# CESSProject/DeOSS

Measured on AMD Instinct MI355X. Metric: device-resident GiB/s hashed to Merkle root; 1/2/4/8 MI355X scaling, higher is better.
Workload: dtype u32; 1 GPU; BASELINE configs[1]: 1 object of 8 GiB (8589934592 B) in 1 chunk-range shard(s) of 8 GiB, chunk 33554432 B (256 leaves); object_bytes=8589934592, chunk=33554432, leaves=256, parallelism=single GPU

## Files before the change

deoss_amd/csrc/merkle_kernels.hpp:

```cpp
#pragma once
#include "quad_ring.hpp"
#include "sha256_gfx950.hpp"

namespace dm {

constexpr int kBlock = 256;
constexpr int kLeafFuseMax = 8;
constexpr int kReduceTile = 512;

struct LeafArgs {
    const uint8_t* base;
    uint64_t pitch;
    uint64_t leaf_len;
    uint64_t last_len;
    const uint64_t* addrs;
    const uint64_t* lens;
    uint64_t nleaves;
    uint64_t byte_off;
    uint64_t byte_end;
    uint32_t* state;
    uint8_t* digests;
    uint8_t* level_out;
    uint32_t fuse_levels;
};
// ... 368 lines not shown
        X7 = t_ + dpp_swap_pairs(y_);                                                  \
    } while (0)

__device__ __forceinline__ void pair_rounds_from_kw(uint32_t (&x)[4], const uint4 (*kw)[kLatLeaves], uint32_t lane,
                                                    uint32_t sh1, uint32_t sh2, uint32_t sh3, uint32_t msk,
                                                    bool lane_b) {
    uint32_t x4 = x[0], x5 = x[1], x6 = x[2], x7 = x[3];
    uint4 q = kw[0][lane];
#pragma unroll
    for (int g = 0; g < 16; g++) {
        uint4 nq = q;
        if (g + 1 < 16) nq = kw[g + 1][lane];
        DM_PAIR_ROUND(x4, x5, x6, x7, q.x);
        DM_PAIR_ROUND(x7, x4, x5, x6, q.y);
        DM_PAIR_ROUND(x6, x7, x4, x5, q.z);
        DM_PAIR_ROUND(x5, x6, x7, x4, q.w);
        q = nq;
    }
    x[0] += x4; x[1] += x5; x[2] += x6; x[3] += x7;
}

template <bool TABLE, bool ALIGNED>
__global__ __launch_bounds__(kLatThreads) void leaf_kernel_pair(LeafArgs a) {
    __shared__ uint4 ring[kLatRing][16][kLatLeaves];
    __shared__ uint32_t lds_a[kPairLeaves][8];
    __shared__ uint32_t lds_b[kPairLeaves / 2][8];
    const uint32_t lane = threadIdx.x & (kLatLeaves - 1);
    const bool producer = __builtin_amdgcn_readfirstlane(threadIdx.x) < kLatLeaves;
    const bool lane_b = (lane & 1) != 0;
    const uint32_t c = lane >> 1;
    const uint64_t first = (uint64_t)blockIdx.x * kPairLeaves;
    const uint64_t i = first + c;
    const LeafView v = leaf_view<TABLE>(a, i);
    const uint64_t NB = wave_max_u64(v.nb);
    if (producer) {
        Blk cur;
        if (v.nb > 0 && !lane_b) cur = load_block<ALIGNED>(v.p);
        for (uint64_t b = 0; b < NB; b++) {
            if (b < v.nb) {
                uint32_t w[16];
                block_words(cur, w);
                if (b + 1 < v.nb && !lane_b) cur = load_block<ALIGNED>(v.p + 64 * (b + 1));
                uint4 (*kw)[kLatLeaves] = ring[b % kLatRing];
#pragma unroll
                for (int q = 0; q < 16; q++) {
                    uint32_t u[4];
#pragma unroll
                    for (int j = 0; j < 4; j++) {
                        const int t = 4 * q + j;
                        uint32_t wt;
                        if (t < 16) {
                            wt = w[t];
                        } else {
                            wt = ssig1(w[(t - 2) & 15]) + w[(t - 7) & 15] + ssig0(w[(t - 15) & 15]) + w[t & 15];
                            w[t & 15] = wt;
                        }
                        u[j] = lane_b ? 0u : kSha256K[t] + wt;
                    }
                    kw[q][lane] = make_uint4(u[0], u[1], u[2], u[3]);
                }
            }
            __syncthreads();
        }
        __syncthreads();
    } else {
        const uint32_t sh1 = lane_b ? 2 : 6, sh2 = lane_b ? 13 : 11, sh3 = lane_b ? 22 : 25;
        const uint32_t msk = lane_b ? 0u : ~0u;
        uint32_t st0[8];
        if (v.active) load_or_init_state(a, i, st0);
        else init_state(st0);
        uint32_t x[4];
#pragma unroll
        for (int k = 0; k < 4; k++) x[k] = lane_b ? st0[k] : st0[4 + k];
        __syncthreads();
        for (uint64_t b = 0; b < NB; b++) {
            if (b < v.nb) pair_rounds_from_kw(x, ring[b % kLatRing], lane, sh1, sh2, sh3, msk, lane_b);
            __syncthreads();
        }
        uint32_t st[8];
#pragma unroll
        for (int k = 0; k < 4; k++) {
            const uint32_t other = dpp_swap_pairs(x[k]);
            st[k] = lane_b ? x[k] : other;
            st[4 + k] = lane_b ? other : x[k];
        }
        if (v.active && !lane_b) {
            leaf_epilogue<ALIGNED>(a, i, v, st);
#pragma unroll
            for (int k = 0; k < 8; k++) lds_a[c][k] = st[k];
        }
    }
    if (a.fuse_levels == 0) return;
    __syncthreads();
    const uint32_t cnt = (uint32_t)((a.nleaves - first) < kPairLeaves ? (a.nleaves - first) : kPairLeaves);
    uint32_t (*res)[8];
    const uint32_t out_cnt = lds_reduce(lds_a, lds_b, cnt, a.fuse_levels, &res);
    if (threadIdx.x < out_cnt) {
        uint32_t o8[8];
#pragma unroll
        for (int k = 0; k < 8; k++) o8[k] = res[threadIdx.x][k];
        const uint64_t o = (uint64_t)blockIdx.x * (kPairLeaves >> a.fuse_levels) + threadIdx.x;
        store_digest(a.level_out + 32 * o, o8);
    }
}

constexpr int kQuadLeaves = 8;
constexpr int kQuadBlocks = 8;
constexpr int kQuadFuseMax = 3;
constexpr int kQuadRow = kQuadLeaves;
constexpr size_t kQuadLdsBytes = sizeof(uint4) * kLatRing * 16 * kQuadBlocks * kQuadRow + 4 * 8 * kQuadLeaves +
                                 4 * 8 * (kQuadLeaves / 2);
static_assert(4 * kQuadLdsBytes <= (160u << 10), "four compact K1Q workgroups must fit a CU's LDS");

#define DM_QS_HEAD(X4, X5, X6)                                                                   \
    "v_alignbit_b32 %[r], %[" X4 "], %[" X4 "], %[sh]\n\t"                                      \
    "v_bitop3_b32 %[f], %[" X4 "], %[" X5 "], %[msk] bitop3:0x1e\n\t"                          \
    "v_bitop3_b32 %[f], %[f], %[" X6 "], %[" X5 "] bitop3:0xca\n\t"                             \
    "v_xor_b32_dpp %[s], %[r], %[r] quad_perm:[1,2,0,3] row_mask:0xf bank_mask:0xf\n\t"
#define DM_QS_SIGMA "v_xor_b32_dpp %[s], %[r], %[s] quad_perm:[2,0,1,3] row_mask:0xf bank_mask:0xf\n\t"
#define DM_QS_STEP_Q(X4, X5, X6, X7, H, HN, VN, QP)                                             \
    DM_QS_HEAD(X4, X5, X6)                                                                       \
    "v_sub_u32_dpp %[" X6 "], %[" VN "], %[" X6 "] quad_perm:" QP " row_mask:0xf bank_mask:0x3\n\t" \
    DM_QS_SIGMA                                                                                  \
    "v_sub_u32_dpp %[" HN "], %[" X4 "], %[" X6 "] row_ror:8 row_mask:0xf bank_mask:0xf\n\t"    \
    "v_add3_u32 %[" X7 "], %[s], %[f], %[" H "]\n\t"
#define DM_QS_STEP(X4, X5, X6, X7, H, HN, VN) DM_QS_STEP_Q(X4, X5, X6, X7, H, HN, VN, "[0,1,2,3]")
#define DM_QS_STEP_A(X4, X5, X6, X7, H, HN)                                                     \
    DM_QS_HEAD(X4, X5, X6)                                                                       \
    DM_QS_SIGMA                                                                                  \
    "v_sub_u32_dpp %[" HN "], %[" X4 "], %[" X6 "] row_ror:8 row_mask:0xf bank_mask:0xf\n\t"    \
    "v_add3_u32 %[" X7 "], %[s], %[f], %[" H "]\n\t"
#define DM_QS_STEP_END(X4, X5, X6, X7, H)                                                       \
    DM_QS_HEAD(X4, X5, X6)                                                                       \
    DM_QS_SIGMA                                                                                  \
    "v_add3_u32 %[" X7 "], %[s], %[f], %[" H "]\n\t"
#define DM_QS_STEPS4V(V0, V1, V2, V3)                                                          \
    DM_QS_STEP("a", "b", "c", "d", "h", "g", V0) DM_QS_STEP("d", "a", "b", "c", "g", "h", V1)   \
    DM_QS_STEP("c", "d", "a", "b", "h", "g", V2) DM_QS_STEP("b", "c", "d", "a", "g", "h", V3)
#define DM_QS_ALIGN_MIS ".p2align 3\n\t.if %[mis]\n\ts_nop 0\n\t.endif\n\t"
#define DM_QS_PROLOGUE(V) DM_QS_PROLOGUE_AT(V, DM_QS_ALIGN_MIS, "[0,1,2,3]")
#define DM_QS_PROLOGUE_AT(V, ALIGN, QP)                                                           \
    "s_nop 1\n\t" ALIGN                                                                          \
    "v_sub_u32_dpp %[d], %[" V "], %[d] quad_perm:" QP " row_mask:0xf bank_mask:0x3\n\t"         \
    "v_sub_u32_dpp %[h], %[b], %[d] row_ror:8 row_mask:0xf bank_mask:0xf\n\t"
#define DM_QS_RESTORE_A(P, X) "v_mov_b32_dpp %[" P "], %[" X "] quad_perm:[0,1,2,3] row_mask:0xf bank_mask:0xc\n\t"
#define DM_QS_GROUP0(V0, V1, V2, V3)                                                             \
    DM_QS_STEP("a", "b", "c", "d", "h", "g", V0) DM_QS_RESTORE_A("d", "x3")                      \
    DM_QS_STEP("d", "a", "b", "c", "g", "h", V1) DM_QS_RESTORE_A("c", "x2")                      \
    DM_QS_STEP("c", "d", "a", "b", "h", "g", V2) DM_QS_STEP("b", "c", "d", "a", "g", "h", V3)
#define DM_QS_FF(X, P, BANKS) "v_add_u32_dpp %[" X "], %[" P "], %[" X "] quad_perm:[0,1,2,3] row_mask:0xf bank_mask:" BANKS "\n\t"
#define DM_QS_TAIL(V0, V1, V2)                                                                   \
    DM_QS_STEP("a", "b", "c", "d", "h", "g", V0) DM_QS_STEP("d", "a", "b", "c", "g", "h", V1)   \
    DM_QS_STEP("c", "d", "a", "b", "h", "g", V2) DM_QS_STEP_A("b", "c", "d", "a", "g", "h")      \
    DM_QS_FF("x3", "d", "0x3") DM_QS_FF("x2", "c", "0x3") DM_QS_FF("x1", "b", "0x3")             \
    DM_QS_FF("x0", "a", "0x3")                                                                   \
    DM_QS_STEP_A("a", "b", "c", "d", "h", "g") DM_QS_STEP_END("d", "a", "b", "c", "g")           \
    DM_QS_FF("x0", "a", "0xc") DM_QS_FF("x1", "b", "0xc") DM_QS_FF("x3", "d", "0xc")             \
    DM_QS_FF("x2", "c", "0xc")
#define DM_QS_STEPS4Q(V0, Q0, V1, Q1, V2, Q2, V3, Q3)                                          \
    DM_QS_STEP_Q("a", "b", "c", "d", "h", "g", V0, Q0) DM_QS_STEP_Q("d", "a", "b", "c", "g", "h", V1, Q1) \
    DM_QS_STEP_Q("c", "d", "a", "b", "h", "g", V2, Q2) DM_QS_STEP_Q("b", "c", "d", "a", "g", "h", V3, Q3)
#define DM_QS_GROUP0Q(V0, Q0, V1, Q1, V2, Q2, V3, Q3)                                          \
    DM_QS_STEP_Q("a", "b", "c", "d", "h", "g", V0, Q0) DM_QS_RESTORE_A("d", "x3")              \
    DM_QS_STEP_Q("d", "a", "b", "c", "g", "h", V1, Q1) DM_QS_RESTORE_A("c", "x2")              \
    DM_QS_STEP_Q("c", "d", "a", "b", "h", "g", V2, Q2) DM_QS_STEP_Q("b", "c", "d", "a", "g", "h", V3, Q3)
#define DM_QS_TAILQ(V0, Q0, V1, Q1, V2, Q2)                                                     \
    DM_QS_STEP_Q("a", "b", "c", "d", "h", "g", V0, Q0) DM_QS_STEP_Q("d", "a", "b", "c", "g", "h", V1, Q1) \
    DM_QS_STEP_Q("c", "d", "a", "b", "h", "g", V2, Q2) DM_QS_STEP_A("b", "c", "d", "a", "g", "h") \
    DM_QS_FF("x3", "d", "0x3") DM_QS_FF("x2", "c", "0x3") DM_QS_FF("x1", "b", "0x3")             \
    DM_QS_FF("x0", "a", "0x3")                                                                   \
    DM_QS_STEP_A("a", "b", "c", "d", "h", "g") DM_QS_STEP_END("d", "a", "b", "c", "g")           \
    DM_QS_FF("x0", "a", "0xc") DM_QS_FF("x1", "b", "0xc") DM_QS_FF("x3", "d", "0xc")             \
    DM_QS_FF("x2", "c", "0xc")
#define DM_QS_OUT                                                                                \
    : [a] "+v"(p0), [b] "+v"(p1), [c] "+v"(p2), [d] "+v"(p3), [h] "+v"(h), [g] "+v"(g),           \
      [x0] "+v"(x[0]), [x1] "+v"(x[1]), [x2] "+v"(x[2]), [x3] "+v"(x[3]), [r] "=&v"(r_),          \
      [f] "=&v"(f_), [s] "=&v"(s_)
#define DM_QS_OPS DM_QS_OUT : [mis] "i"(MIS ? 1 : 0), [sh] "v"(sh.x), [msk] "v"(msk), [v0] "v"(v0), [v1] "v"(v1), [v2] "v"(v2), [v3] "v"(v3)

template <bool MIS, class KW>
__device__ __forceinline__ void quad_block_skewed(uint32_t (&x)[4], KW kw, uint3 sh, uint32_t msk) {
    uint32_t p0 = x[0], p1 = x[1], p2 = x[2], p3 = x[3], h = 0, g = 0, r_, f_, s_;
    uint4 q = kw(0), nq = kw(1);
    {
        const uint32_t v0 = q.x, v1 = 0, v2 = 0, v3 = 0;
        asm volatile(DM_QS_PROLOGUE("v0") DM_QS_OPS);
    }
#pragma unroll
    for (int grp = 0; grp < 16; grp++) {
        const uint4 nnq = grp + 2 < 16 ? kw(grp + 2) : nq;
        const uint32_t v0 = q.y, v1 = q.z, v2 = q.w, v3 = nq.x;
        if (grp == 0) {
            asm volatile(DM_QS_ALIGN_MIS DM_QS_GROUP0("v0", "v1", "v2", "v3") DM_QS_OPS);
        } else if (grp < 15) {
            asm volatile(DM_QS_ALIGN_MIS DM_QS_STEPS4V("v0", "v1", "v2", "v3") DM_QS_OPS);
        } else {
            asm volatile(DM_QS_ALIGN_MIS DM_QS_TAIL("v0", "v1", "v2") DM_QS_OPS);
        }
        q = nq;
        nq = nnq;
    }
}

constexpr int kLgkmWait0 = 0xC07F;

#define DM_QS_HNB(HN, A, B, BANKS) "v_sub_u32_dpp %[" HN "], %[" A "], %[" B "] row_ror:8 row_mask:0xf bank_mask:" BANKS "\n\t"
#define DM_QS_ADDB(D, A, B, BANKS) "v_add_u32_dpp %[" D "], %[" A "], %[" B "] quad_perm:[0,1,2,3] row_mask:0xf bank_mask:" BANKS "\n\t"
#define DM_QS_MOVB(D, S, BANKS) "v_mov_b32_dpp %[" D "], %[" S "] quad_perm:[0,1,2,3] row_mask:0xf bank_mask:" BANKS "\n\t"
#define DM_QS_KWN(X6, S, N) "v_sub_u32_dpp %[" X6 "], %[" N "], %[" S "] quad_perm:[0,0,0,0] row_mask:0xf bank_mask:0x3\n\t"
#define DM_QS_ADD3(X7, H) "v_add3_u32 %[" X7 "], %[s], %[f], %[" H "]\n\t"
#define DM_QS_LINKQ(V0, Q0, V1, Q1, V2, Q2, N0, N1, N2)                                          \
    DM_QS_STEP_Q("a", "b", "c", "d", "h", "g", V0, Q0) DM_QS_STEP_Q("d", "a", "b", "c", "g", "h", V1, Q1) \
    DM_QS_STEP_Q("c", "d", "a", "b", "h", "g", V2, Q2)                                           \
    DM_QS_ADDB("x1", "x1", "b", "0xc") DM_QS_ADDB("x3", "x3", "d", "0x3")                        \
                                            \
    DM_QS_HEAD("b", "c", "d") DM_QS_KWN("d", "x3", N0) DM_QS_SIGMA                               \
    DM_QS_HNB("h", "x1", "d", "0x3") DM_QS_HNB("h", "b", "d", "0xc") DM_QS_ADD3("a", "g")        \
    DM_QS_ADDB("b", "x1", "b", "0x3") DM_QS_ADDB("c", "x2", "c", "0x3")                          \
    DM_QS_HNB("g", "a", "c", "0xc") DM_QS_ADDB("x0", "x0", "a", "0xc")                           \
    DM_QS_ADDB("a", "a", "x0", "0x3") DM_QS_MOVB("x2", "c", "0x3")                               \
                                                            \
    DM_QS_HEAD("a", "b", "c") DM_QS_KWN("c", "c", N1) DM_QS_SIGMA                                \
    DM_QS_HNB("g", "x0", "c", "0x3") DM_QS_ADD3("d", "h")                                        \
    DM_QS_ADDB("x3", "x3", "d", "0xc") DM_QS_MOVB("x1", "b", "0x3") DM_QS_MOVB("x0", "a", "0x3") \
                                           \
    DM_QS_HEAD("d", "a", "b") DM_QS_KWN("b", "b", N2) DM_QS_SIGMA                                \
    DM_QS_HNB("h", "x3", "b", "0x3") DM_QS_HNB("h", "d", "x1", "0xc") DM_QS_ADD3("c", "g")       \
    DM_QS_ADDB("x2", "x2", "c", "0xc") DM_QS_MOVB("a", "x0", "0xc") DM_QS_MOVB("d", "x3", "0xc") \
    DM_QS_MOVB("c", "x2", "0xc")
#define DM_QS_BODYQ                                                                              \
    DM_QS_STEPS4Q("q01", "[1,1,1,1]", "q02", "[1,1,1,1]", "q03", "[1,1,1,1]", "q00", "[2,2,2,2]") \
    DM_QS_STEPS4Q("q01", "[2,2,2,2]", "q02", "[2,2,2,2]", "q03", "[2,2,2,2]", "q00", "[3,3,3,3]") \
    DM_QS_STEPS4Q("q01", "[3,3,3,3]", "q02", "[3,3,3,3]", "q03", "[3,3,3,3]", "q10", "[0,0,0,0]") \
    DM_QS_STEPS4Q("q11", "[0,0,0,0]", "q12", "[0,0,0,0]", "q13", "[0,0,0,0]", "q10", "[1,1,1,1]") \
    DM_QS_STEPS4Q("q11", "[1,1,1,1]", "q12", "[1,1,1,1]", "q13", "[1,1,1,1]", "q10", "[2,2,2,2]") \
    DM_QS_STEPS4Q("q11", "[2,2,2,2]", "q12", "[2,2,2,2]", "q13", "[2,2,2,2]", "q10", "[3,3,3,3]") \
    DM_QS_STEPS4Q("q11", "[3,3,3,3]", "q12", "[3,3,3,3]", "q13", "[3,3,3,3]", "q20", "[0,0,0,0]") \
    DM_QS_STEPS4Q("q21", "[0,0,0,0]", "q22", "[0,0,0,0]", "q23", "[0,0,0,0]", "q20", "[1,1,1,1]") \
    DM_QS_STEPS4Q("q21", "[1,1,1,1]", "q22", "[1,1,1,1]", "q23", "[1,1,1,1]", "q20", "[2,2,2,2]") \
    DM_QS_STEPS4Q("q21", "[2,2,2,2]", "q22", "[2,2,2,2]", "q23", "[2,2,2,2]", "q20", "[3,3,3,3]") \
    DM_QS_STEPS4Q("q21", "[3,3,3,3]", "q22", "[3,3,3,3]", "q23", "[3,3,3,3]", "q30", "[0,0,0,0]") \
    DM_QS_STEPS4Q("q31", "[0,0,0,0]", "q32", "[0,0,0,0]", "q33", "[0,0,0,0]", "q30", "[1,1,1,1]") \
    DM_QS_STEPS4Q("q31", "[1,1,1,1]", "q32", "[1,1,1,1]", "q33", "[1,1,1,1]", "q30", "[2,2,2,2]") \
    DM_QS_STEPS4Q("q31", "[2,2,2,2]", "q32", "[2,2,2,2]", "q33", "[2,2,2,2]", "q30", "[3,3,3,3]")
#define DM_QS_FILLQ                                                                              \
    DM_QS_PROLOGUE_AT("q00", DM_QS_ALIGN_MIS, "[0,0,0,0]")                                       \
    DM_QS_GROUP0Q("q01", "[0,0,0,0]", "q02", "[0,0,0,0]", "q03", "[0,0,0,0]", "q00", "[1,1,1,1]")
#define DM_QS_CONTQ                                                                              \
    DM_QS_ALIGN_MIS                                                                              \
    DM_QS_STEP_Q("c", "d", "a", "b", "h", "g", "q03", "[0,0,0,0]") DM_QS_STEP_Q("b", "c", "d", "a", "g", "h", "q00", "[1,1,1,1]")
#define DM_QS_ENDLINKQ DM_QS_LINKQ("q31", "[3,3,3,3]", "q32", "[3,3,3,3]", "q33", "[3,3,3,3]", "n0", "n1", "n2")
#define DM_QS_ENDTAILQ DM_QS_TAILQ("q31", "[3,3,3,3]", "q32", "[3,3,3,3]", "q33", "[3,3,3,3]")
#define DM_QS_STATE [a] "+v"(P[0]), [b] "+v"(P[1]), [c] "+v"(P[2]), [d] "+v"(P[3]),              \
                    [x0] "+v"(x[0]), [x1] "+v"(x[1]), [x2] "+v"(x[2]), [x3] "+v"(x[3]),           \
                    [r] "=&v"(r_), [f] "=&v"(f_), [s] "=&v"(s_)
#define DM_QS_KIN [mis] "i"(MIS ? 1 : 0), [sh] "v"(sh.x), [msk] "v"(msk),                        \
                  [q00] "v"(K[0].x), [q01] "v"(K[0].y), [q02] "v"(K[0].z), [q03] "v"(K[0].w),     \
                  [q10] "v"(K[1].x), [q11] "v"(K[1].y), [q12] "v"(K[1].z), [q13] "v"(K[1].w),     \
                  [q20] "v"(K[2].x), [q21] "v"(K[2].y), [q22] "v"(K[2].z), [q23] "v"(K[2].w),     \
                  [q30] "v"(K[3].x), [q31] "v"(K[3].y), [q32] "v"(K[3].z), [q33] "v"(K[3].w)

template <bool MIS, int K8>
__device__ __forceinline__ void quad_block_regs(uint32_t (&x)[4], uint32_t (&P)[4], uint32_t& h, uint32_t& g,
                                                const uint4 (&K)[4], const uint4& N, uint3 sh, uint32_t msk) {
    uint32_t r_, f_, s_;
    if constexpr (K8 == 0) {
        asm volatile(DM_QS_FILLQ DM_QS_BODYQ DM_QS_ENDLINKQ
                     : DM_QS_STATE, [h] "=&v"(h), [g] "=&v"(g)
                     : DM_QS_KIN, [n0] "v"(N.x), [n1] "v"(N.y), [n2] "v"(N.z));
    } else if constexpr (K8 < kQuadBlocks - 1) {
        asm volatile(DM_QS_CONTQ DM_QS_BODYQ DM_QS_ENDLINKQ
                     : DM_QS_STATE, [h] "+v"(h), [g] "+v"(g)
                     : DM_QS_KIN, [n0] "v"(N.x), [n1] "v"(N.y), [n2] "v"(N.z));
    } else {
        asm volatile(DM_QS_CONTQ DM_QS_BODYQ DM_QS_ENDTAILQ
                     : DM_QS_STATE, [h] "+v"(h), [g] "+v"(g)
                     : DM_QS_KIN);
    }
}

template <int G, int ROW, bool MIS, int K8 = 0>
__device__ __forceinline__ void quad_stage_blocks(uint32_t (&x)[4], uint32_t (&P)[4], uint32_t& h, uint32_t& g,
                                                  uint4 (&S)[3][4], const uint4* kw, uint3 sh, uint32_t msk) {
    __builtin_amdgcn_s_waitcnt(kLgkmWait0);
    if constexpr (K8 + 2 < kQuadBlocks) {
#pragma unroll
        for (int t = 0; t < 4; t++) S[(K8 + 2) % 3][t] = kw[(K8 + 2) * ROW + 4 * t * G];
    }
    quad_block_regs<MIS, K8>(x, P, h, g, S[K8 % 3], S[(K8 + 1) % 3][0], sh, msk);
    if constexpr (K8 + 1 < kQuadBlocks) quad_stage_blocks<G, ROW, MIS, K8 + 1>(x, P, h, g, S, kw, sh, msk);
}
template <int G, int ROW, bool MIS>
__device__ __forceinline__ void quad_stage_regs(uint32_t (&x)[4], const uint4* kw, uint3 sh, uint32_t msk) {
    uint4 S[3][4];
    uint32_t P[4] = {x[0], x[1], x[2], x[3]}, h, g;
#pragma unroll
    for (int k = 0; k < 2; k++) {
#pragma unroll
        for (int t = 0; t < 4; t++) S[k][t] = kw[k * ROW + 4 * t * G];
    }
    quad_stage_blocks<G, ROW, MIS>(x, P, h, g, S, kw, sh, msk);
}

constexpr int kQuadWideRing = quad_ring::kWideDepth;
constexpr int kQuadSets = quad_ring::kSets;
template <int G, int ROW, int K8, bool FILL, bool TAIL, bool LOAD>
__device__ __forceinline__ void quad_xstage_block(uint32_t (&x)[4], uint32_t (&P)[4], uint32_t& h, uint32_t& g,
                                                  uint4 (&S)[kQuadSets][4], const uint4* src, uint3 sh, uint32_t msk) {
    static_assert((LOAD || !quad_ring::block_prefetches(K8, true)) && (!TAIL || !quad_ring::block_links(K8, true)) &&
                      !(FILL && TAIL) && quad_ring::prefetch_of(K8).block == (K8 + quad_ring::kAhead) % kQuadBlocks,
                  "only the last stage of a run skips a load or drains: quad_ring.hpp");
    __builtin_amdgcn_s_waitcnt(kLgkmWait0);
    if constexpr (LOAD) {
        constexpr quad_ring::BlockRef pf = quad_ring::prefetch_of(K8);
#pragma unroll
        for (int t = 0; t < 4; t++) S[quad_ring::set_of(K8 + quad_ring::kAhead)][t] = src[pf.block * ROW + 4 * t * G];
    }
    quad_block_regs<false, FILL ? 0 : TAIL ? kQuadBlocks - 1 : 1>(x, P, h, g, S[quad_ring::set_of(K8)],
                                                                 S[quad_ring::set_of(K8 + 1)][0], sh, msk);
}
template <int G, int ROW>
__device__ __forceinline__ uint32_t quad_run_xstage(uint32_t (&x)[4], const uint4* colp, uint32_t slot, uint64_t n,
                                                    uint3 sh, uint32_t msk) {
    uint4 S[kQuadSets][4];
    uint32_t P[4] = {x[0], x[1], x[2], x[3]}, h, g;
    const uint4* cur = colp + slot * 16 * G;
#pragma unroll
    for (int k = 0; k < quad_ring::kAhead; k++) {
#pragma unroll
        for (int t = 0; t < 4; t++) S[k][t] = cur[k * ROW + 4 * t * G];
    }
    quad_xstage_block<G, ROW, 0, true, false, true>(x, P, h, g, S, cur, sh, msk);
    for (uint64_t s = 1; s < n; s++) {
        slot = quad_ring::next_slot(slot, kQuadWideRing);
        const uint4* nxt = colp + slot * 16 * G;
        quad_xstage_block<G, ROW, 1, false, false, true>(x, P, h, g, S, cur, sh, msk);
        quad_xstage_block<G, ROW, 2, false, false, true>(x, P, h, g, S, cur, sh, msk);
        quad_xstage_block<G, ROW, 3, false, false, true>(x, P, h, g, S, cur, sh, msk);
        quad_xstage_block<G, ROW, 4, false, false, true>(x, P, h, g, S, cur, sh, msk);
        quad_xstage_block<G, ROW, 5, false, false, true>(x, P, h, g, S, cur, sh, msk);
        quad_xstage_block<G, ROW, 6, false, false, true>(x, P, h, g, S, nxt, sh, msk);
        quad_xstage_block<G, ROW, 7, false, false, true>(x, P, h, g, S, nxt, sh, msk);
        __syncthreads();
        quad_xstage_block<G, ROW, 0, false, false, true>(x, P, h, g, S, nxt, sh, msk);
        cur = nxt;
    }
    quad_xstage_block<G, ROW, 1, false, false, true>(x, P, h, g, S, cur, sh, msk);
    quad_xstage_block<G, ROW, 2, false, false, true>(x, P, h, g, S, cur, sh, msk);
    quad_xstage_block<G, ROW, 3, false, false, true>(x, P, h, g, S, cur, sh, msk);
    quad_xstage_block<G, ROW, 4, false, false, true>(x, P, h, g, S, cur, sh, msk);
    quad_xstage_block<G, ROW, 5, false, false, true>(x, P, h, g, S, cur, sh, msk);
    quad_xstage_block<G, ROW, 6, false, false, false>(x, P, h, g, S, cur, sh, msk);
    quad_xstage_block<G, ROW, 7, false, true, false>(x, P, h, g, S, cur, sh, msk);
    __syncthreads();
    return quad_ring::next_slot(slot, kQuadWideRing);
}

template <bool ALIGNED, int G>
__device__ __forceinline__ void quad_produce_block(const LeafView& v, Blk& cur, uint64_t b, uint4* kw) {
    if (b >= v.nb) return;
    uint32_t w[16];
    block_words(cur, w);
    if (b + kQuadBlocks < v.nb) cur = load_block<ALIGNED>(v.p + 64 * (b + kQuadBlocks));
#pragma unroll
    for (int q = 0; q < 16; q++) {
        uint32_t u[4];
#pragma unroll
        for (int k = 0; k < 4; k++) {
            const int t = 4 * q + k;
            uint32_t wt;
            if (t < 16) {
                wt = w[t];
            } else {
                wt = ssig1(w[(t - 2) & 15]) + w[(t - 7) & 15] + ssig0(w[(t - 15) & 15]) + w[t & 15];
                w[t & 15] = wt;
            }
            u[k] = 0u - (kSha256K[t] + wt);
        }
        kw[q * G] = make_uint4(u[0], u[1], u[2], u[3]);
    }
}

template <bool TABLE, bool ALIGNED, bool COMPACT>
__global__ __launch_bounds__(kLatThreads) void leaf_kernel_quad(LeafArgs a) {
    constexpr int ROW = COMPACT ? kQuadRow : kQuadLeaves;
    constexpr int G = kQuadBlocks * ROW;
    constexpr int DEPTH = COMPACT ? kLatRing : kQuadWideRing;
    __shared__ uint4 ring[COMPACT ? 1 : 2][kLatRing][16][G];
    __shared__ uint32_t lds_a[kQuadLeaves][8];
    __shared__ uint32_t lds_b[kQuadLeaves / 2][8];
    static_assert(DEPTH * sizeof(ring[0][0]) <= sizeof(ring), "the ring's stages must fit its LDS");
    static_assert(COMPACT || (3 * sizeof(ring) > (160u << 10) && sizeof(ring) <= (64u << 10) &&
                              2 * (sizeof(ring) + sizeof(lds_a) + sizeof(lds_b)) <= (160u << 10)),
                  "the wide K1Q must stay at exactly two workgroups per CU (160 KiB of LDS)");
    const uint32_t lane = threadIdx.x & 63;
    const bool producer = __builtin_amdgcn_readfirstlane(threadIdx.x) < 64;
    const uint32_t c = lane >> 3;
    const uint32_t j = lane & 7;
    const uint64_t first = (uint64_t)blockIdx.x * kQuadLeaves;
    const uint64_t i = first + c;
    const LeafView v = leaf_view<TABLE>(a, i);
    const uint64_t NB = wave_max_u64(v.nb);
    const uint64_t NI = (NB + kQuadBlocks - 1) / kQuadBlocks;
    if (producer) {
        Blk cur;
        if (j < v.nb) cur = load_block<ALIGNED>(v.p + 64 * j);
        if constexpr (!COMPACT) {
            uint4* const kw0 = &ring[0][0][0][j * ROW + c];
            uint32_t slot = 0;
            for (uint64_t s = 0; s < quad_ring::stages_before_first_barrier(DEPTH); s++) {
                if (s < NI) quad_produce_block<ALIGNED, G>(v, cur, s * kQuadBlocks + j, kw0 + slot * 16 * G);
                slot = quad_ring::next_slot(slot, DEPTH);
            }
            __syncthreads();
            for (uint64_t it = 0; it < NI; it++) {
                const uint64_t s = quad_ring::stage_written_after_barrier(it, DEPTH);
                if (s < NI) quad_produce_block<ALIGNED, G>(v, cur, s * kQuadBlocks + j, kw0 + slot * 16 * G);
                slot = quad_ring::next_slot(slot, DEPTH);
                __syncthreads();
            }
        } else {
            for (uint64_t it = 0; it < NI; it++) {
                const uint64_t b = it * kQuadBlocks + j;
                if (b < v.nb) {
                    uint32_t w[16];
                    block_words(cur, w);
                    if (b + kQuadBlocks < v.nb) cur = load_block<ALIGNED>(v.p + 64 * (b + kQuadBlocks));
                    uint4* kw = &ring[0][it % kLatRing][0][j * ROW + c];
#pragma unroll
                    for (int q = 0; q < 16; q++) {
                        uint32_t u[4];
#pragma unroll
                        for (int k = 0; k < 4; k++) {
                            const int t = 4 * q + k;
                            uint32_t wt;
                            if (t < 16) {
                                wt = w[t];
                            } else {
                                wt = ssig1(w[(t - 2) & 15]) + w[(t - 7) & 15] + ssig0(w[(t - 15) & 15]) + w[t & 15];
                                w[t & 15] = wt;
                            }
                            u[k] = 0u - (kSha256K[t] + wt);
                        }
                        kw[q * G] = make_uint4(u[0], u[1], u[2], u[3]);
                    }
                }
                __syncthreads();
            }
            __syncthreads();
        }
    } else {
        __builtin_amdgcn_s_setprio(1);
        const uint32_t cq = 2 * (lane >> 4) + ((lane >> 2) & 1);
        const bool role_a = (lane >> 3) & 1;
        const uint32_t p = lane & 3;
        const uint64_t iq = first + cq;
        const LeafView vq = leaf_view<TABLE>(a, iq);
        const uint3 sh = make_uint3(role_a ? (p == 0 ? 2 : p == 1 ? 13 : 22) : (p == 0 ? 6 : p == 1 ? 11 : 25), 0, 0);
        const uint32_t msk = role_a ? 0u : ~0u;
        uint32_t st0[8];
        if (vq.active) load_or_init_state(a, iq, st0);
        else init_state(st0);
        uint32_t x[4];
#pragma unroll
        for (int k = 0; k < 4; k++) x[k] = role_a ? st0[(k + 2) & 3] : st0[4 + k];
        const uint4* col = &ring[0][0][0][cq];
        __syncthreads();
        uint32_t xf[4];
#pragma unroll
        for (int k = 0; k < 4; k++) xf[k] = x[k];
        const uint64_t NS = uniform_u64(NI);
        uint32_t wslot = 0;
        for (uint64_t it = 0; it < NS;) {
            const bool running = COMPACT ? vq.active && vq.nb > it * kQuadBlocks
                                         : quad_ring::leaf_running(vq.active, vq.nb, it);
            const uint64_t end = uniform_u64(wave_min_u64(COMPACT ? (running ? vq.nb / kQuadBlocks : NS)
                                                                  : quad_ring::leaf_run_end(running, vq.nb, NS)));
            if constexpr (COMPACT) {
                for (; it < end; it++) {
                    quad_stage_regs<G, ROW, COMPACT>(x, col + (it % kLatRing) * 16 * G + p * G, sh, msk);
                    __syncthreads();
                }
            } else if (it < end) {
                wslot = quad_run_xstage<G, ROW>(x, col + p * G, wslot, end - it, sh, msk);
                it = end;
            }
            if (running) {
#pragma unroll
                for (int k = 0; k < 4; k++) xf[k] = x[k];
            }
            if (it == NS) break;
            if (!__any(COMPACT ? vq.active && vq.nb > it * kQuadBlocks && vq.nb < (it + 1) * kQuadBlocks
                               : quad_ring::leaf_ends_inside(vq.active, vq.nb, it)))
                continue;
            const uint4* kw = col + (COMPACT ? (uint32_t)(it % kLatRing) : wslot) * 16 * G;
            const uint64_t b0 = it * kQuadBlocks;
            for (uint32_t k = 0; k < kQuadBlocks; k++) {
                const uint4* kb = kw + k * ROW;
                if (b0 + k < vq.nb)
                    quad_block_skewed<COMPACT>(x, [kb](int g) { return kb[g * G]; }, sh, msk);
            }
            if (vq.nb > b0) {
#pragma unroll
                for (int k = 0; k < 4; k++) xf[k] = x[k];
            }
            __syncthreads();
            it++;
            wslot = quad_ring::next_slot(wslot, DEPTH);
        }
        uint32_t st[8];
#pragma unroll
        for (int k = 0; k < 4; k++) {
            st[k] = __shfl(xf[(k + 2) & 3], (int)(lane + 8), 64);
            st[4 + k] = xf[k];
        }
        if (vq.active && !role_a && p == 0) {
            leaf_epilogue<ALIGNED>(a, iq, vq, st);
#pragma unroll
            for (int k = 0; k < 8; k++) lds_a[cq][k] = st[k];
        }
    }
    if (a.fuse_levels == 0) return;
    __syncthreads();
    const uint32_t cnt = (uint32_t)((a.nleaves - first) < kQuadLeaves ? (a.nleaves - first) : kQuadLeaves);
    uint32_t (*res)[8];
    const uint32_t out_cnt = lds_reduce(lds_a, lds_b, cnt, a.fuse_levels, &res);
    if (threadIdx.x < out_cnt) {
        uint32_t o8[8];
#pragma unroll
        for (int k = 0; k < 8; k++) o8[k] = res[threadIdx.x][k];
        const uint64_t o = (uint64_t)blockIdx.x * (kQuadLeaves >> a.fuse_levels) + threadIdx.x;
        store_digest(a.level_out + 32 * o, o8);
    }
}

__global__ __launch_bounds__(kLatThreads) void quad_shape_primer(int x) {
    extern __shared__ uint4 dyn[];
    if (x == 12345) dyn[threadIdx.x] = make_uint4(1, 1, 1, 1);
}

__global__ __launch_bounds__(kBlock) void reduce_kernel(const uint8_t* in, uint64_t m, uint32_t levels,
                                                         uint8_t* out) {
    __shared__ uint32_t lds_a[kBlock][8];
    __shared__ uint32_t lds_b[kBlock / 2][8];
    const uint64_t base = (uint64_t)blockIdx.x * kReduceTile;
    const uint32_t cnt = (uint32_t)((m - base) < kReduceTile ? (m - base) : kReduceTile);
    const uint32_t t = threadIdx.x;
    const uint32_t next = (cnt + 1) >> 1;
    if (t < next) {
        uint32_t L[8], R[8], o[8];
        const uint32_t ri = (2 * t + 1 < cnt) ? 2 * t + 1 : cnt - 1;
        load_digest(in + 32 * (base + 2 * t), L);
        load_digest(in + 32 * (base + ri), R);
        node_hash(L, R, o);
#pragma unroll
        for (int k = 0; k < 8; k++) lds_a[t][k] = o[k];
    }
    __syncthreads();
    uint32_t (*res)[8];
    const uint32_t out_cnt = lds_reduce(lds_a, lds_b, next, levels - 1, &res);
    if (t < out_cnt) {
        uint32_t v[8];
#pragma unroll
        for (int k = 0; k < 8; k++) v[k] = res[t][k];
        store_digest(out + 32 * ((uint64_t)blockIdx.x * (kReduceTile >> levels) + t), v);
    }
}

__global__ __launch_bounds__(kBlock) void batch_root_kernel(const uint8_t* leaves, const uint64_t* leaf_first,
                                                             const uint32_t* obj_ids, uint8_t* roots) {
    __shared__ uint32_t lds_a[kBlock][8];
    __shared__ uint32_t lds_b[kBlock / 2][8];
    const uint32_t o = obj_ids[blockIdx.x];
    const uint64_t base = leaf_first[o];
    const uint32_t cnt = (uint32_t)(leaf_first[o + 1] - base);
    const uint32_t t = threadIdx.x;
    const uint32_t next = (cnt + 1) >> 1;
    if (t < next) {
        uint32_t L[8], R[8], h[8];
        const uint32_t ri = (2 * t + 1 < cnt) ? 2 * t + 1 : cnt - 1;
        load_digest(leaves + 32 * (base + 2 * t), L);
        load_digest(leaves + 32 * (base + ri), R);
        node_hash(L, R, h);
#pragma unroll
        for (int k = 0; k < 8; k++) lds_a[t][k] = h[k];
    }
    __syncthreads();
    uint32_t levels = 0;
    for (uint32_t c = next; c > 1; c = (c + 1) >> 1) levels++;
    uint32_t (*res)[8];
    lds_reduce(lds_a, lds_b, next, levels, &res);
    if (t == 0) {
        uint32_t v[8];
#pragma unroll
        for (int k = 0; k < 8; k++) v[k] = res[0][k];
        store_digest(roots + 32 * (uint64_t)o, v);
    }
}

__device__ __forceinline__ uint64_t splitmix64(uint64_t z) {
    z += 0x9e3779b97f4a7c15ULL;
    z = (z ^ (z >> 30)) * 0xbf58476d1ce4e5b9ULL;
    z = (z ^ (z >> 27)) * 0x94d049bb133111ebULL;
    return z ^ (z >> 31);
}

__global__ __launch_bounds__(kBlock) void fill_splitmix_kernel(uint64_t* dst, uint64_t word0, uint64_t nwords,
                                                                uint64_t seed) {
    const uint64_t stride = (uint64_t)gridDim.x * kBlock * 2;
    for (uint64_t j = ((uint64_t)blockIdx.x * kBlock + threadIdx.x) * 2; j < nwords; j += stride) {
        if (j + 1 < nwords) {
            ulonglong2 v = make_ulonglong2(splitmix64(seed ^ (word0 + j)), splitmix64(seed ^ (word0 + j + 1)));
            *reinterpret_cast<ulonglong2*>(dst + j) = v;
        } else {
            dst[j] = splitmix64(seed ^ (word0 + j));
        }
    }
}

constexpr int kProbeLoads = 16;
__global__ __launch_bounds__(kBlock) void read_probe_kernel(const uint8_t* p, uint64_t n16, uint64_t* out) {
    const u32x4_t* g = reinterpret_cast<const u32x4_t*>(p);
    const uint64_t per = (n16 + gridDim.x - 1) / gridDim.x;
    const uint64_t lo = (uint64_t)blockIdx.x * per, hi = lo + per < n16 ? lo + per : n16;
    u32x4_t acc[kProbeLoads];
#pragma unroll
    for (int u = 0; u < kProbeLoads; u++) acc[u] = u32x4_t{0u, 0u, 0u, 0u};
    uint64_t i = lo + threadIdx.x;
    for (; i + (kProbeLoads - 1) * kBlock < hi; i += kProbeLoads * kBlock) {
        u32x4_t x[kProbeLoads];
#pragma unroll
        for (int u = 0; u < kProbeLoads; u++) x[u] = __builtin_nontemporal_load(g + i + u * kBlock);
#pragma unroll
        for (int u = 0; u < kProbeLoads; u++) acc[u] ^= x[u];
    }
    for (; i < hi; i += kBlock) acc[0] ^= g[i];
#pragma unroll
    for (int u = 1; u < kProbeLoads; u++) acc[0] ^= acc[u];
    uint64_t v = (((uint64_t)acc[0].y << 32) | acc[0].x) ^ (((uint64_t)acc[0].w << 32) | acc[0].z);
    for (int m = 32; m >= 1; m >>= 1) v ^= __shfl_xor(v, m, 64);
    __shared__ uint64_t part[kBlock / 64];
    if ((threadIdx.x & 63) == 0) part[threadIdx.x >> 6] = v;
    __syncthreads();
    if (threadIdx.x == 0) {
        uint64_t t = 0;
        for (int w = 0; w < kBlock / 64; w++) t ^= part[w];
        atomicXor(reinterpret_cast<unsigned long long*>(out), (unsigned long long)t);
    }
}

}
```

Baseline: 16.94 GiB/s.

## Alternate state register sets across blocks in wide quad SHA stage to drop moves

New measurement: 17.09 GiB/s (median of 6 runs). About the same (+0.9%).

```diff
diff --git a/deoss_amd/csrc/merkle_kernels.hpp b/deoss_amd/csrc/merkle_kernels.hpp
--- a/deoss_amd/csrc/merkle_kernels.hpp
+++ b/deoss_amd/csrc/merkle_kernels.hpp
@@ -694,11 +694,107 @@
     quad_stage_blocks<G, ROW, MIS>(x, P, h, g, S, kw, sh, msk);
 }
 
+#define DM_QS_LINKW(F0, F1, F2, F3, W0, W1, W2, W3, D0, D1, E0, E1, V0, Q0, V1, Q1, V2, Q2, N0, N1, N2) \
+    DM_QS_STEP_Q(F0, F1, F2, F3, "h", "g", V0, Q0) DM_QS_STEP_Q(F3, F0, F1, F2, "g", "h", V1, Q1) \
+    DM_QS_STEP_Q(F2, F3, F0, F1, "h", "g", V2, Q2)                                               \
+    DM_QS_ADDB("t", "t", F1, "0xc")                                                              \
+                                            \
+    DM_QS_HEAD(F1, F2, F3) DM_QS_ADDB(F3, W3, F3, "0x3") DM_QS_KWN(W3, F3, N0) DM_QS_SIGMA       \
+    DM_QS_HNB("h", "t", W3, "0x3") DM_QS_HNB("h", F1, F3, "0xc") DM_QS_ADD3(F0, "g")             \
+    DM_QS_ADDB(F1, W1, F1, "0x3") DM_QS_ADDB(F2, W2, F2, "0x3")                                  \
+    DM_QS_HNB("g", F0, F2, "0xc") DM_QS_ADDB(F0, W0, F0, "0x3")                                  \
+                                                            \
+    DM_QS_HEAD(F0, F1, F2) DM_QS_KWN(W3, F2, N1) DM_QS_SIGMA DM_QS_ADD3(E0, "h")                 \
+                                           \
+    DM_QS_HEAD(E0, F0, F1) DM_QS_ADDB(F0, W0, F0, "0xc") DM_QS_ADDB(E0, D0, E0, "0xc")           \
+    DM_QS_KWN("t", F1, N2) DM_QS_SIGMA                                                           \
+    DM_QS_HNB("g", F0, W3, "0x3") DM_QS_HNB("h", E0, "t", "0xf") DM_QS_ADD3(E1, "g")             \
+    DM_QS_ADDB(E1, D1, E1, "0xc")
+#define DM_QS_CONTW(N0, N1, O0, D0, D1)                                                          \
+    DM_QS_ALIGN_MIS                                                                              \
+    DM_QS_HEAD(D1, D0, O0)                                                                       \
+    "v_sub_u32_dpp %[" N0 "], %[q03], %[" O0 "] quad_perm:[0,0,0,0] row_mask:0xf bank_mask:0x3\n\t" \
+    DM_QS_SIGMA DM_QS_HNB("g", D1, N0, "0x3") DM_QS_HNB("g", D1, O0, "0xc") DM_QS_ADD3(N1, "h")  \
+    DM_QS_STEP_Q(N1, D1, D0, N0, "g", "h", "q00", "[1,1,1,1]")
+#define DM_QS_STEPS4N(N0, N1, N2, N3, C4, V0, Q0, V1, Q1, V2, Q2, V3, Q3)                      \
+    DM_QS_STEP_Q(N0, N1, C4, N3, "h", "g", V0, Q0) DM_QS_STEP_Q(N3, N0, N1, N2, "g", "h", V1, Q1) \
+    DM_QS_STEP_Q(N2, N3, N0, N1, "h", "g", V2, Q2) DM_QS_STEP_Q(N1, N2, N3, N0, "g", "h", V3, Q3)
+#define DM_QS_BODYW(N0, N1, N2, N3, C4)                                                          \
+    DM_QS_STEPS4N(N0, N1, N2, N3, C4, "q01", "[1,1,1,1]", "q02", "[1,1,1,1]", "q03", "[1,1,1,1]", "q00", "[2,2,2,2]") \
+    DM_QS_STEPS4N(N0, N1, N2, N3, N2, "q01", "[2,2,2,2]", "q02", "[2,2,2,2]", "q03", "[2,2,2,2]", "q00", "[3,3,3,3]") \
+    DM_QS_STEPS4N(N0, N1, N2, N3, N2, "q01", "[3,3,3,3]", "q02", "[3,3,3,3]", "q03", "[3,3,3,3]", "q10", "[0,0,0,0]") \
+    DM_QS_STEPS4N(N0, N1, N2, N3, N2, "q11", "[0,0,0,0]", "q12", "[0,0,0,0]", "q13", "[0,0,0,0]", "q10", "[1,1,1,1]") \
+    DM_QS_STEPS4N(N0, N1, N2, N3, N2, "q11", "[1,1,1,1]", "q12", "[1,1,1,1]", "q13", "[1,1,1,1]", "q10", "[2,2,2,2]") \
+    DM_QS_STEPS4N(N0, N1, N2, N3, N2, "q11", "[2,2,2,2]", "q12", "[2,2,2,2]", "q13", "[2,2,2,2]", "q10", "[3,3,3,3]") \
+    DM_QS_STEPS4N(N0, N1, N2, N3, N2, "q11", "[3,3,3,3]", "q12", "[3,3,3,3]", "q13", "[3,3,3,3]", "q20", "[0,0,0,0]") \
+    DM_QS_STEPS4N(N0, N1, N2, N3, N2, "q21", "[0,0,0,0]", "q22", "[0,0,0,0]", "q23", "[0,0,0,0]", "q20", "[1,1,1,1]") \
+    DM_QS_STEPS4N(N0, N1, N2, N3, N2, "q21", "[1,1,1,1]", "q22", "[1,1,1,1]", "q23", "[1,1,1,1]", "q20", "[2,2,2,2]") \
+    DM_QS_STEPS4N(N0, N1, N2, N3, N2, "q21", "[2,2,2,2]", "q22", "[2,2,2,2]", "q23", "[2,2,2,2]", "q20", "[3,3,3,3]") \
+    DM_QS_STEPS4N(N0, N1, N2, N3, N2, "q21", "[3,3,3,3]", "q22", "[3,3,3,3]", "q23", "[3,3,3,3]", "q30", "[0,0,0,0]") \
+    DM_QS_STEPS4N(N0, N1, N2, N3, N2, "q31", "[0,0,0,0]", "q32", "[0,0,0,0]", "q33", "[0,0,0,0]", "q30", "[1,1,1,1]") \
+    DM_QS_STEPS4N(N0, N1, N2, N3, N2, "q31", "[1,1,1,1]", "q32", "[1,1,1,1]", "q33", "[1,1,1,1]", "q30", "[2,2,2,2]") \
+    DM_QS_STEPS4N(N0, N1, N2, N3, N2, "q31", "[2,2,2,2]", "q32", "[2,2,2,2]", "q33", "[2,2,2,2]", "q30", "[3,3,3,3]")
+#define DM_QS_TAILW_ODD(F0, F1, F2, F3, W0, W1, W2, W3, D0, D1, V0, Q0, V1, Q1, V2, Q2)           \
+    DM_QS_STEP_Q(F0, F1, F2, F3, "h", "g", V0, Q0) DM_QS_STEP_Q(F3, F0, F1, F2, "g", "h", V1, Q1) \
+    DM_QS_STEP_Q(F2, F3, F0, F1, "h", "g", V2, Q2) DM_QS_STEP_A(F1, F2, F3, F0, "g", "h")        \
+    DM_QS_ADDB(F3, W3, F3, "0x3") DM_QS_ADDB(F2, W2, F2, "0x3") DM_QS_ADDB(F1, W1, F1, "0x3")    \
+    DM_QS_HNB("g", F0, F2, "0xc") DM_QS_ADDB(F0, W0, F0, "0x3")                                  \
+    DM_QS_STEP_END(F0, F1, F2, W3, "h") DM_QS_STEP_END(W3, F0, F1, W2, "g")                      \
+    DM_QS_ADDB(F0, W0, F0, "0xc") DM_QS_ADDB(F1, "t", F1, "0xc") DM_QS_ADDB(F3, D0, W3, "0xc")   \
+    DM_QS_ADDB(F2, D1, W2, "0xc")
+#define DM_QS_TAILW_EVEN(D0, D1, V0, Q0, V1, Q1, V2, Q2)                                         \
+    DM_QS_STEP_Q("a", "b", "c", "d", "h", "g", V0, Q0) DM_QS_STEP_Q("d", "a", "b", "c", "g", "h", V1, Q1) \
+    DM_QS_STEP_Q("c", "d", "a", "b", "h", "g", V2, Q2) DM_QS_STEP_A("b", "c", "d", "a", "g", "h") \
+    DM_QS_FF("x3", "d", "0x3") DM_QS_FF("x2", "c", "0x3") DM_QS_FF("x1", "b", "0x3")             \
+    DM_QS_FF("x0", "a", "0x3")                                                                   \
+    DM_QS_STEP_A("a", "b", "c", "d", "h", "g") DM_QS_STEP_END("d", "a", "b", "c", "g")           \
+    DM_QS_FF("x0", "a", "0xc") DM_QS_ADDB("x1", "b", "t", "0xc") DM_QS_ADDB("x3", "d", D0, "0xc") \
+    DM_QS_ADDB("x2", D1, "c", "0xc")
+#define DM_QS_W_FILL DM_QS_FILLQ DM_QS_BODYW("a", "b", "c", "d", "c")                                    \
+    DM_QS_LINKW("a", "b", "c", "d", "x0", "x1", "x2", "x3", "z0", "z1", "y0", "y1", "q31", "[3,3,3,3]", "q32", "[3,3,3,3]", "q33", "[3,3,3,3]", "n0", "n1", "n2")
+#define DM_QS_W_EVEN DM_QS_CONTW("a", "b", "x0", "z0", "z1") DM_QS_BODYW("a", "b", "c", "d", "z1")      \
+    DM_QS_LINKW("a", "b", "c", "d", "x0", "x1", "x2", "x3", "z0", "z1", "y0", "y1", "q31", "[3,3,3,3]", "q32", "[3,3,3,3]", "q33", "[3,3,3,3]", "n0", "n1", "n2")
+#define DM_QS_W_ODD DM_QS_CONTW("x0", "x1", "a", "y0", "y1") DM_QS_BODYW("x0", "x1", "x2", "x3", "y1")      \
+    DM_QS_LINKW("x0", "x1", "x2", "x3", "a", "b", "c", "d", "y0", "y1", "z0", "z1", "q31", "[3,3,3,3]", "q32", "[3,3,3,3]", "q33", "[3,3,3,3]", "n0", "n1", "n2")
+#define DM_QS_W_ODD_TAIL DM_QS_CONTW("x0", "x1", "a", "y0", "y1") DM_QS_BODYW("x0", "x1", "x2", "x3", "y1") \
+    DM_QS_TAILW_ODD("x0", "x1", "x2", "x3", "a", "b", "c", "d", "y0", "y1", "q31", "[3,3,3,3]", "q32", "[3,3,3,3]", "q33", "[3,3,3,3]")
+#define DM_QS_W_EVEN_TAIL DM_QS_CONTW("a", "b", "x0", "z0", "z1") DM_QS_BODYW("a", "b", "c", "d", "z1") \
+    DM_QS_TAILW_EVEN("z0", "z1", "q31", "[3,3,3,3]", "q32", "[3,3,3,3]", "q33", "[3,3,3,3]")
+#define DM_QS_STATEW DM_QS_STATE, [y0] "+v"(Y[0]), [y1] "+v"(Y[1]), [z0] "+v"(Z[0]),             \
+                     [z1] "+v"(Z[1]), [t] "+v"(t)
+
+template <int K8, bool FILL, bool TAIL>
+__device__ __forceinline__ void quad_block_alt(uint32_t (&x)[4], uint32_t (&P)[4], uint32_t (&Y)[2], uint32_t (&Z)[2],
+                                               uint32_t& t, uint32_t& h, uint32_t& g, const uint4 (&K)[4],
+                                               const uint4& N, uint3 sh, uint32_t msk) {
+    static_assert(!(FILL && (K8 & 1)) && !(TAIL && !(K8 & 1)), "a run is whole stages: it fills even, drains odd");
+    constexpr bool MIS = false;
+    uint32_t r_, f_, s_;
+    if constexpr (FILL) {
+        asm volatile(DM_QS_W_FILL
+                     : DM_QS_STATEW, [h] "=&v"(h), [g] "=&v"(g)
+                     : DM_QS_KIN, [n0] "v"(N.x), [n1] "v"(N.y), [n2] "v"(N.z));
+    } else if constexpr (TAIL) {
+        asm volatile(DM_QS_W_ODD_TAIL
+                     : DM_QS_STATEW, [h] "+v"(h), [g] "+v"(g)
+                     : DM_QS_KIN);
+    } else if constexpr (K8 & 1) {
+        asm volatile(DM_QS_W_ODD
+                     : DM_QS_STATEW, [h] "+v"(h), [g] "+v"(g)
+                     : DM_QS_KIN, [n0] "v"(N.x), [n1] "v"(N.y), [n2] "v"(N.z));
+    } else {
+        asm volatile(DM_QS_W_EVEN
+                     : DM_QS_STATEW, [h] "+v"(h), [g] "+v"(g)
+                     : DM_QS_KIN, [n0] "v"(N.x), [n1] "v"(N.y), [n2] "v"(N.z));
+    }
+}
+
 constexpr int kQuadWideRing = quad_ring::kWideDepth;
 constexpr int kQuadSets = quad_ring::kSets;
 template <int G, int ROW, int K8, bool FILL, bool TAIL, bool LOAD>
-__device__ __forceinline__ void quad_xstage_block(uint32_t (&x)[4], uint32_t (&P)[4], uint32_t& h, uint32_t& g,
-                                                  uint4 (&S)[kQuadSets][4], const uint4* src, uint3 sh, uint32_t msk) {
+__device__ __forceinline__ void quad_xstage_block(uint32_t (&x)[4], uint32_t (&P)[4], uint32_t (&Y)[2], uint32_t (&Z)[2],
+                                                  uint32_t& t, uint32_t& h, uint32_t& g, uint4 (&S)[kQuadSets][4],
+                                                  const uint4* src, uint3 sh, uint32_t msk) {
     static_assert((LOAD || !quad_ring::block_prefetches(K8, true)) && (!TAIL || !quad_ring::block_links(K8, true)) &&
                       !(FILL && TAIL) && quad_ring::prefetch_of(K8).block == (K8 + quad_ring::kAhead) % kQuadBlocks,
                   "only the last stage of a run skips a load or drains: quad_ring.hpp");
@@ -708,42 +804,43 @@
 #pragma unroll
         for (int t = 0; t < 4; t++) S[quad_ring::set_of(K8 + quad_ring::kAhead)][t] = src[pf.block * ROW + 4 * t * G];
     }
-    quad_block_regs<false, FILL ? 0 : TAIL ? kQuadBlocks - 1 : 1>(x, P, h, g, S[quad_ring::set_of(K8)],
-                                                                 S[quad_ring::set_of(K8 + 1)][0], sh, msk);
+    quad_block_alt<K8, FILL, TAIL>(x, P, Y, Z, t, h, g, S[quad_ring::set_of(K8)], S[quad_ring::set_of(K8 + 1)][0], sh,
+                                   msk);
 }
 template <int G, int ROW>
 __device__ __forceinline__ uint32_t quad_run_xstage(uint32_t (&x)[4], const uint4* colp, uint32_t slot, uint64_t n,
                                                     uint3 sh, uint32_t msk) {
     uint4 S[kQuadSets][4];
     uint32_t P[4] = {x[0], x[1], x[2], x[3]}, h, g;
+    uint32_t t = x[1], Z[2] = {x[3], x[2]}, Y[2] = {x[3], x[2]};
     const uint4* cur = colp + slot * 16 * G;
 #pragma unroll
     for (int k = 0; k < quad_ring::kAhead; k++) {
 #pragma unroll
         for (int t = 0; t < 4; t++) S[k][t] = cur[k * ROW + 4 * t * G];
     }
-    quad_xstage_block<G, ROW, 0, true, false, true>(x, P, h, g, S, cur, sh, msk);
+    quad_xstage_block<G, ROW, 0, true, false, true>(x, P, Y, Z, t, h, g, S, cur, sh, msk);
     for (uint64_t s = 1; s < n; s++) {
         slot = quad_ring::next_slot(slot, kQuadWideRing);
         const uint4* nxt = colp + slot * 16 * G;
-        quad_xstage_block<G, ROW, 1, false, false, true>(x, P, h, g, S, cur, sh, msk);
-        quad_xstage_block<G, ROW, 2, false, false, true>(x, P, h, g, S, cur, sh, msk);
-        quad_xstage_block<G, ROW, 3, false, false, true>(x, P, h, g, S, cur, sh, msk);
-        quad_xstage_block<G, ROW, 4, false, false, true>(x, P, h, g, S, cur, sh, msk);
-        quad_xstage_block<G, ROW, 5, false, false, true>(x, P, h, g, S, cur, sh, msk);
-        quad_xstage_block<G, ROW, 6, false, false, true>(x, P, h, g, S, nxt, sh, msk);
-        quad_xstage_block<G, ROW, 7, false, false, true>(x, P, h, g, S, nxt, sh, msk);
+        quad_xstage_block<G, ROW, 1, false, false, true>(x, P, Y, Z, t, h, g, S, cur, sh, msk);
+        quad_xstage_block<G, ROW, 2, false, false, true>(x, P, Y, Z, t, h, g, S, cur, sh, msk);
+        quad_xstage_block<G, ROW, 3, false, false, true>(x, P, Y, Z, t, h, g, S, cur, sh, msk);
+        quad_xstage_block<G, ROW, 4, false, false, true>(x, P, Y, Z, t, h, g, S, cur, sh, msk);
+        quad_xstage_block<G, ROW, 5, false, false, true>(x, P, Y, Z, t, h, g, S, cur, sh, msk);
+        quad_xstage_block<G, ROW, 6, false, false, true>(x, P, Y, Z, t, h, g, S, nxt, sh, msk);
+        quad_xstage_block<G, ROW, 7, false, false, true>(x, P, Y, Z, t, h, g, S, nxt, sh, msk);
         __syncthreads();
-        quad_xstage_block<G, ROW, 0, false, false, true>(x, P, h, g, S, nxt, sh, msk);
+        quad_xstage_block<G, ROW, 0, false, false, true>(x, P, Y, Z, t, h, g, S, nxt, sh, msk);
         cur = nxt;
     }
-    quad_xstage_block<G, ROW, 1, false, false, true>(x, P, h, g, S, cur, sh, msk);
-    quad_xstage_block<G, ROW, 2, false, false, true>(x, P, h, g, S, cur, sh, msk);
-    quad_xstage_block<G, ROW, 3, false, false, true>(x, P, h, g, S, cur, sh, msk);
-    quad_xstage_block<G, ROW, 4, false, false, true>(x, P, h, g, S, cur, sh, msk);
-    quad_xstage_block<G, ROW, 5, false, false, true>(x, P, h, g, S, cur, sh, msk);
-    quad_xstage_block<G, ROW, 6, false, false, false>(x, P, h, g, S, cur, sh, msk);
-    quad_xstage_block<G, ROW, 7, false, true, false>(x, P, h, g, S, cur, sh, msk);
+    quad_xstage_block<G, ROW, 1, false, false, true>(x, P, Y, Z, t, h, g, S, cur, sh, msk);
+    quad_xstage_block<G, ROW, 2, false, false, true>(x, P, Y, Z, t, h, g, S, cur, sh, msk);
+    quad_xstage_block<G, ROW, 3, false, false, true>(x, P, Y, Z, t, h, g, S, cur, sh, msk);
+    quad_xstage_block<G, ROW, 4, false, false, true>(x, P, Y, Z, t, h, g, S, cur, sh, msk);
+    quad_xstage_block<G, ROW, 5, false, false, true>(x, P, Y, Z, t, h, g, S, cur, sh, msk);
+    quad_xstage_block<G, ROW, 6, false, false, false>(x, P, Y, Z, t, h, g, S, cur, sh, msk);
+    quad_xstage_block<G, ROW, 7, false, true, false>(x, P, Y, Z, t, h, g, S, cur, sh, msk);
     __syncthreads();
     return quad_ring::next_slot(slot, kQuadWideRing);
 }
```
